# eric-zqwang/puzzlefusion-plusplus

Hardware: AMD Instinct MI355X
Metric: denoiser DDPM-step throughput (fragment*steps/s) (higher is better)
Workload: dtype f32 (GEMMs: f16x3); 1 GPU; DDPM training iteration, BASELINE configs[1]: add_noise + rotate + frozen PointNet++/VQ encode (in the loop) + DenoiserTransformer forward (dropouts on) + MSE + full backward + [encoder of iteration i+1 issued on its own stream during iteration i] AdamW; padded_slots=not evaluated (their gradient contribution is exactly zero), puzzles_per_gpu=32, fragment_slots=20, points_per_fragment=1024, valid_fragments_per_gpu=154, weights=random init, reference architecture (57.6M denoiser + 0.6M encoder params)

## Files before the change

### puzzlefusion-plusplus_amd/csrc/sa_train.hip

```cpp
#include <hip/hip_runtime.h>
#include <stdint.h>

#include "gemm_common.h"
#include "pfpp.h"
#include "pfpp_common.h"
#include "sa_common.h"

namespace {

struct SaTP {
  const float* xyz; const float* ctr; const float* feats; const int32_t* idx;
  const _Float16* wh[3]; const _Float16* wl[3];
  const float* bias[3];
  const float* am[2]; const float* aa[2];
  double* stats; int copies;
  float* y_out; float* out_max; float* out_min;
  int N, S, G;
  const float* u; int D;
  _Float16* e_hi; _Float16* e_lo;
  const int32_t* sched;
};

struct PadWalk {
  const int32_t* order;
  int G, n2, S, i, ib;
  __device__ __forceinline__ PadWalk(const int32_t* sched, int G_, int k, int S_) : order(sched), G(G_), S(S_), i(k) {
    n2 = sched ? sched[G_] : G_;
    const int r = n2 % S_;
    ib = n2 + (k >= r ? k - r : k - r + S_);
    if (i >= n2) i = ib;
  }
  __device__ __forceinline__ bool two() const { return i < n2; }
  __device__ __forceinline__ int cnt() const { return (order && i < G) ? order[2 * G + 1 + i] : 64; }
  __device__ __forceinline__ int g() const { return i < G ? (order ? order[i] : i) : G; }
  __device__ __forceinline__ void next() {
    const int j = i + S;
    i = (i < n2 && j >= n2) ? ib : j;
  }
};

__device__ __forceinline__ f32x16 bn_train_relu_t(const f32x16 acc, const float* B, const float* M, const float* A, int c0, int lhi) {
  f32x16 y;
#pragma unroll
  for (int q = 0; q < 4; ++q) {
    const float4 b4 = *reinterpret_cast<const float4*>(B + c0 + 8 * q + 4 * lhi);
    const float4 m4 = *reinterpret_cast<const float4*>(M + c0 + 8 * q + 4 * lhi);
    const float4 a4 = *reinterpret_cast<const float4*>(A + c0 + 8 * q + 4 * lhi);
    const float bv[4] = {b4.x, b4.y, b4.z, b4.w}, mv[4] = {m4.x, m4.y, m4.z, m4.w}, av[4] = {a4.x, a4.y, a4.z, a4.w};
#pragma unroll
    for (int r = 0; r < 4; ++r) {
      const float v = __builtin_fmaf(acc[4 * q + r] + bv[r], mv[r], av[r]);
      y[4 * q + r] = v > 0.0f ? v : 0.0f;
    }
  }
  return y;
}

__device__ __forceinline__ void flush_stats(double* stats, int copies, int C, int c, int lhi, double s, double q) {
  const double a = s + __shfl_xor(s, 32), b = q + __shfl_xor(q, 32);
  if (lhi == 0) {
    double* st = stats + (size_t)((blockIdx.x * 4 + (threadIdx.x >> 6)) % copies) * 2 * C;
    unsafeAtomicAdd(st + c, a);
    unsafeAtomicAdd(st + C + c, b);
  }
}

template <int C1, int C2, int C3, int STAGE>
__global__ __launch_bounds__(256, 1) void sa1_train_kernel(const SaTP p) {
  constexpr int CS = STAGE == 1 ? C1 : (STAGE == 2 ? C2 : C3);
  constexpr int NT1 = C1 / 32, NT2 = STAGE >= 2 ? C2 / 32 : 1, NT3 = STAGE >= 3 ? C3 / 32 : 1;
  __shared__ __align__(16) float B0[C1], M0[C1], A0[C1], B1[C2], M1[C2], A1[C2];
  constexpr bool LDS_SUMS = STAGE == 3;
  __shared__ double SUMS[LDS_SUMS ? 2 * (CS / 32) : 1][LDS_SUMS ? 256 : 1];
  const int tid = threadIdx.x;
  if (LDS_SUMS)
    for (int i = 0; i < 2 * (CS / 32); ++i) SUMS[i][tid] = 0.0;
  if (STAGE >= 2)
    for (int i = tid; i < C1; i += 256) { B0[i] = p.bias[0][i]; M0[i] = p.am[0][i]; A0[i] = p.aa[0][i]; }
  if (STAGE >= 3)
    for (int i = tid; i < C2; i += 256) { B1[i] = p.bias[1][i]; M1[i] = p.am[1][i]; A1[i] = p.aa[1][i]; }
  __syncthreads();

  const int lane = tid & 63, wave = tid >> 6;
  const int l31 = lane & 31, lhi = lane >> 5;

  half8 w0h[NT1], w0l[NT1];
  half8 w1h[NT2][C1 / 16], w1l[NT2][C1 / 16];
  half8 w2h[NT3][C2 / 16], w2l[NT3][C2 / 16];
#pragma unroll
  for (int t = 0; t < NT1; ++t) {
#pragma unroll
    for (int q = 0; q < 8; ++q) { w0h[t][q] = (_Float16)0.0f; w0l[t][q] = (_Float16)0.0f; }
    if (lhi == 0) {
      w0h[t] = *reinterpret_cast<const half8*>(p.wh[0] + (t * 32 + l31) * 8);
      w0l[t] = *reinterpret_cast<const half8*>(p.wl[0] + (t * 32 + l31) * 8);
    }
  }
  if (STAGE >= 2) {
#pragma unroll
    for (int t = 0; t < NT2; ++t)
#pragma unroll
      for (int ks = 0; ks < C1 / 16; ++ks) {
        w1h[t][ks] = *reinterpret_cast<const half8*>(p.wh[1] + (t * 32 + l31) * C1 + ks * 16 + lhi * 8);
        w1l[t][ks] = *reinterpret_cast<const half8*>(p.wl[1] + (t * 32 + l31) * C1 + ks * 16 + lhi * 8);
      }
  }
  if (STAGE >= 3) {
#pragma unroll
    for (int n = 0; n < NT3; ++n)
#pragma unroll
      for (int ks = 0; ks < C2 / 16; ++ks) {
        w2h[n][ks] = *reinterpret_cast<const half8*>(p.wh[2] + (n * 32 + l31) * C2 + ks * 16 + lhi * 8);
        w2l[n][ks] = *reinterpret_cast<const half8*>(p.wl[2] + (n * 32 + l31) * C2 + ks * 16 + lhi * 8);
      }
  }
  float bs[CS / 32];
  double ss[CS / 32], sq[CS / 32];
#pragma unroll
  for (int n = 0; n < CS / 32; ++n) { bs[n] = p.bias[STAGE - 1][n * 32 + l31]; ss[n] = 0.0; sq[n] = 0.0; }

  auto stat = [&](const f32x16& acc, int n, int g) {
    float s = 0.0f, q = 0.0f, mx = -__builtin_huge_valf(), mn = __builtin_huge_valf();
#pragma unroll
    for (int e = 0; e < 16; ++e) {
      const float y = acc[e] + bs[n];
      s += y;
      q = __builtin_fmaf(y, y, q);
      if (STAGE == 3) { mx = fmaxf(mx, y); mn = fminf(mn, y); }
    }
    if (LDS_SUMS) {
      SUMS[2 * n][tid] += (double)s;
      SUMS[2 * n + 1][tid] += (double)q;
    } else {
      ss[n] += (double)s;
      sq[n] += (double)q;
    }
    if (STAGE == 3) {
      mx = fmaxf(mx, __shfl_xor(mx, 32));
      mn = fminf(mn, __shfl_xor(mn, 32));
      if (lhi == 0) {
        p.out_max[(int64_t)g * C3 + n * 32 + l31] = mx;
        p.out_min[(int64_t)g * C3 + n * 32 + l31] = mn;
      }
    }
  };

  const int stride = gridDim.x * 4;
  const int g0 = blockIdx.x * 4 + wave;
  auto load_id = [&](int g) {
    const int gc = g < p.G ? g : p.G - 1;
    const int id = p.idx[(int64_t)gc * 32 + l31];
    return id < p.N ? id : p.N - 1;
  };
  auto load_pt = [&](int g, int id, float (&q)[3], float (&c)[3]) {
    const int gc = g < p.G ? g : p.G - 1;
    const int f = gc / p.S;
    const float* q3 = p.xyz + ((int64_t)f * p.N + id) * 3;
    const float* c3 = p.ctr + (int64_t)gc * 3;
#pragma unroll
    for (int d = 0; d < 3; ++d) { q[d] = q3[d]; c[d] = c3[d]; }
  };
  float q_cur[3], c_cur[3], q_nxt[3], c_nxt[3];
  int id_nxt;
  load_pt(g0, load_id(g0), q_cur, c_cur);
  id_nxt = load_id(g0 + stride);

  for (int g = g0; g < p.G; g += stride) {
    load_pt(g + stride, id_nxt, q_nxt, c_nxt);
    id_nxt = load_id(g + 2 * stride);

    half8 xh, xl;
#pragma unroll
    for (int q = 0; q < 8; ++q) { xh[q] = (_Float16)0.0f; xl[q] = (_Float16)0.0f; }
    if (lhi == 0) {
#pragma unroll
      for (int d = 0; d < 3; ++d) {
        _Float16 a, b;
        split1(__fsub_rn(q_cur[d], c_cur[d]), a, b);
        xh[d] = a; xl[d] = b;
      }
    }

    if (STAGE == 1) {
#pragma unroll
      for (int n = 0; n < NT1; ++n) {
        f32x16 acc;
#pragma unroll
        for (int e = 0; e < 16; ++e) acc[e] = 0.0f;
        acc = __builtin_amdgcn_mfma_f32_32x32x16_f16(xl, w0h[n], acc, 0, 0, 0);
        acc = __builtin_amdgcn_mfma_f32_32x32x16_f16(xh, w0l[n], acc, 0, 0, 0);
        acc = __builtin_amdgcn_mfma_f32_32x32x16_f16(xh, w0h[n], acc, 0, 0, 0);
        stat(acc, n, g);
      }
    } else {
      half8 f1h[C1 / 16], f1l[C1 / 16];
#pragma unroll
      for (int t = 0; t < NT1; ++t) {
        f32x16 acc;
#pragma unroll
        for (int e = 0; e < 16; ++e) acc[e] = 0.0f;
        acc = __builtin_amdgcn_mfma_f32_32x32x16_f16(w0h[t], xl, acc, 0, 0, 0);
        acc = __builtin_amdgcn_mfma_f32_32x32x16_f16(w0l[t], xh, acc, 0, 0, 0);
        acc = __builtin_amdgcn_mfma_f32_32x32x16_f16(w0h[t], xh, acc, 0, 0, 0);
        const f32x16 y = bn_train_relu_t(acc, B0, M0, A0, t * 32, lhi);
        half8 fh[2], fl[2];
        tile_to_fragments(y, lhi, fh, fl);
        f1h[2 * t] = fh[0]; f1h[2 * t + 1] = fh[1];
        f1l[2 * t] = fl[0]; f1l[2 * t + 1] = fl[1];
      }
      if (STAGE == 2) {
#pragma unroll
        for (int n = 0; n < NT2; ++n) {
          f32x16 acc;
#pragma unroll
          for (int e = 0; e < 16; ++e) acc[e] = 0.0f;
#pragma unroll
          for (int ks = 0; ks < C1 / 16; ++ks) {
            acc = __builtin_amdgcn_mfma_f32_32x32x16_f16(f1l[ks], w1h[n][ks], acc, 0, 0, 0);
            acc = __builtin_amdgcn_mfma_f32_32x32x16_f16(f1h[ks], w1l[n][ks], acc, 0, 0, 0);
            acc = __builtin_amdgcn_mfma_f32_32x32x16_f16(f1h[ks], w1h[n][ks], acc, 0, 0, 0);
          }
          stat(acc, n, g);
        }
      } else {
        asm volatile("" ::: "memory");
        half8 f2h[C2 / 16], f2l[C2 / 16];
#pragma unroll
        for (int t = 0; t < NT2; ++t) {
          f32x16 acc;
#pragma unroll
          for (int e = 0; e < 16; ++e) acc[e] = 0.0f;
#pragma unroll
          for (int ks = 0; ks < C1 / 16; ++ks) {
            acc = __builtin_amdgcn_mfma_f32_32x32x16_f16(w1h[t][ks], f1l[ks], acc, 0, 0, 0);
            acc = __builtin_amdgcn_mfma_f32_32x32x16_f16(w1l[t][ks], f1h[ks], acc, 0, 0, 0);
            acc = __builtin_amdgcn_mfma_f32_32x32x16_f16(w1h[t][ks], f1h[ks], acc, 0, 0, 0);
          }
          const f32x16 y = bn_train_relu_t(acc, B1, M1, A1, t * 32, lhi);
          half8 fh[2], fl[2];
          tile_to_fragments(y, lhi, fh, fl);
          f2h[2 * t] = fh[0]; f2h[2 * t + 1] = fh[1];
          f2l[2 * t] = fl[0]; f2l[2 * t + 1] = fl[1];
        }
#pragma unroll
        for (int n = 0; n < NT3; ++n) {
          f32x16 acc;
#pragma unroll
          for (int e = 0; e < 16; ++e) acc[e] = 0.0f;
#pragma unroll
          for (int ks = 0; ks < C2 / 16; ++ks) {
            acc = __builtin_amdgcn_mfma_f32_32x32x16_f16(f2l[ks], w2h[n][ks], acc, 0, 0, 0);
            acc = __builtin_amdgcn_mfma_f32_32x32x16_f16(f2h[ks], w2l[n][ks], acc, 0, 0, 0);
            acc = __builtin_amdgcn_mfma_f32_32x32x16_f16(f2h[ks], w2h[n][ks], acc, 0, 0, 0);
          }
          stat(acc, n, g);
        }
      }
    }
#pragma unroll
    for (int d = 0; d < 3; ++d) { q_cur[d] = q_nxt[d]; c_cur[d] = c_nxt[d]; }
  }
#pragma unroll
  for (int n = 0; n < CS / 32; ++n)
    flush_stats(p.stats, p.copies, CS, n * 32 + l31, lhi, LDS_SUMS ? SUMS[LDS_SUMS ? 2 * n : 0][LDS_SUMS ? tid : 0] : ss[n],
                LDS_SUMS ? SUMS[LDS_SUMS ? 2 * n + 1 : 0][LDS_SUMS ? tid : 0] : sq[n]);
}

template <int D, int C1, int C2, int STAGE>
__global__ __launch_bounds__(256, 1) void sa2_train_kernel(const SaTP p) {
  constexpr int KS0 = D / 16 + 1;
  constexpr int KP0 = D + 8;
  constexpr int LD0 = KS0 * 16 + 8, LD1 = C1 + 8;
  constexpr int CS = STAGE == 1 ? C1 : C2;
  extern __shared__ __align__(16) unsigned char sa2t_smem[];
  _Float16* W0h = reinterpret_cast<_Float16*>(sa2t_smem);
  _Float16* W0l = W0h + C1 * LD0;
  _Float16* W1h = W0l + C1 * LD0;
  _Float16* W1l = W1h + C2 * LD1;
  float* B0 = reinterpret_cast<float*>(W1l + C2 * LD1);
  float* M0 = B0 + C1;
  float* A0 = M0 + C1;

  const int tid = threadIdx.x;
  for (int i = tid; i < C1 * (LD0 / 8); i += 256) {
    const int r = i / (LD0 / 8), c8 = i - r * (LD0 / 8);
    uint4 vh = make_uint4(0, 0, 0, 0), vl = vh;
    if (c8 * 8 < KP0) {
      vh = *reinterpret_cast<const uint4*>(p.wh[0] + (size_t)r * KP0 + c8 * 8);
      vl = *reinterpret_cast<const uint4*>(p.wl[0] + (size_t)r * KP0 + c8 * 8);
    }
    *reinterpret_cast<uint4*>(W0h + r * LD0 + c8 * 8) = vh;
    *reinterpret_cast<uint4*>(W0l + r * LD0 + c8 * 8) = vl;
  }
  if (STAGE == 2) {
    for (int i = tid; i < C2 * (C1 / 8); i += 256) {
      const int r = i / (C1 / 8), c8 = i - r * (C1 / 8);
      *reinterpret_cast<uint4*>(W1h + r * LD1 + c8 * 8) = *reinterpret_cast<const uint4*>(p.wh[1] + (size_t)r * C1 + c8 * 8);
      *reinterpret_cast<uint4*>(W1l + r * LD1 + c8 * 8) = *reinterpret_cast<const uint4*>(p.wl[1] + (size_t)r * C1 + c8 * 8);
    }
    for (int i = tid; i < C1; i += 256) { B0[i] = p.bias[0][i]; M0[i] = p.am[0][i]; A0[i] = p.aa[0][i]; }
  }
  __syncthreads();

  const int lane = tid & 63, wave = tid >> 6;
  const int l31 = lane & 31, lhi = lane >> 5;

  float bs[CS / 32];
  double ss[CS / 32], sq[CS / 32];
#pragma unroll
  for (int n = 0; n < CS / 32; ++n) { bs[n] = p.bias[STAGE - 1][n * 32 + l31]; ss[n] = 0.0; sq[n] = 0.0; }

  auto split8 = [&](const float4 a, const float4 b, half8& hi, half8& lo) {
    const float x[8] = {a.x, a.y, a.z, a.w, b.x, b.y, b.z, b.w};
#pragma unroll
    for (int q = 0; q < 8; ++q) {
      _Float16 h, l;
      split1(x[q], h, l);
      hi[q] = h; lo[q] = l;
    }
  };

  const int stride = gridDim.x * 4;
  const int g0 = blockIdx.x * 4 + wave;
  auto load_ids = [&](int g, int (&id)[2]) {
    const int gc = g < p.G ? g : p.G - 1;
#pragma unroll
    for (int st = 0; st < 2; ++st) {
      const int v = p.idx[(int64_t)gc * 64 + st * 32 + l31];
      id[st] = v < p.N ? v : p.N - 1;
    }
  };
  auto load_rows = [&](int g, const int (&id)[2], float4 (&raw)[2][D / 16][2], float (&q)[2][3], float (&c)[3]) {
    const int gc = g < p.G ? g : p.G - 1;
    const int f = gc / p.S;
#pragma unroll
    for (int st = 0; st < 2; ++st) {
// ... 179 lines not shown
#pragma unroll
    for (int ks = 0; ks < K / 16; ++ks) {
      raw[ks][0] = *reinterpret_cast<const float4*>(row + ks * 16);
      raw[ks][1] = *reinterpret_cast<const float4*>(row + ks * 16 + 4);
    }
  };
  float4 raw[K / 16][2];
  PadWalk wk(p.sched, p.G, g0, stride);
  int g = wk.g(), c = wk.cnt(); wk.next();
  int g1 = wk.g(), c1 = wk.cnt(); wk.next();
  int g2 = wk.g(), c2 = wk.cnt();
  load_rows(g, 0, c, raw);
  float mx[N / 32], mn[N / 32];

  for (; g < p.G; g = g1, c = c1, g1 = g2, c1 = c2, wk.next(), g2 = wk.g(), c2 = wk.cnt()) {
    const int nh = c > 32 ? 2 : 1;
#pragma unroll 1
    for (int h = 0; h < nh; ++h) {
      asm volatile("" ::: "memory");
      half8 fh[K / 16], fl[K / 16];
#pragma unroll
      for (int ks = 0; ks < K / 16; ++ks) {
        const float4 m0 = *reinterpret_cast<const float4*>(M + ks * 16 + lhi * 8), m1 = *reinterpret_cast<const float4*>(M + ks * 16 + lhi * 8 + 4);
        const float4 a0 = *reinterpret_cast<const float4*>(A + ks * 16 + lhi * 8), a1 = *reinterpret_cast<const float4*>(A + ks * 16 + lhi * 8 + 4);
        const float mv[8] = {m0.x, m0.y, m0.z, m0.w, m1.x, m1.y, m1.z, m1.w}, av[8] = {a0.x, a0.y, a0.z, a0.w, a1.x, a1.y, a1.z, a1.w};
        const float4 r0 = raw[ks][0], r1 = raw[ks][1];
        const float x[8] = {r0.x, r0.y, r0.z, r0.w, r1.x, r1.y, r1.z, r1.w};
#pragma unroll
        for (int q = 0; q < 8; ++q) {
          const float v = fmaxf(__builtin_fmaf(x[q], mv[q], av[q]), 0.0f);
          _Float16 hh, ll;
          split1(v, hh, ll);
          fh[ks][q] = hh; fl[ks][q] = ll;
        }
      }
      if (h + 1 < nh) load_rows(g, 1, c, raw);
      else load_rows(g1, 0, c1, raw);
#pragma unroll 1
      for (int n = 0; n < N / 32; ++n) {
        f32x16 acc;
#pragma unroll
        for (int e = 0; e < 16; ++e) acc[e] = 0.0f;
#pragma unroll
        for (int ks = 0; ks < K / 16; ++ks) {
          const half8 wh = *reinterpret_cast<const half8*>(Wh + (n * 32 + l31) * LD + ks * 16 + lhi * 8);
          const half8 wl = *reinterpret_cast<const half8*>(Wl + (n * 32 + l31) * LD + ks * 16 + lhi * 8);
          acc = __builtin_amdgcn_mfma_f32_32x32x16_f16(fl[ks], wh, acc, 0, 0, 0);
          acc = __builtin_amdgcn_mfma_f32_32x32x16_f16(fh[ks], wl, acc, 0, 0, 0);
          acc = __builtin_amdgcn_mfma_f32_32x32x16_f16(fh[ks], wh, acc, 0, 0, 0);
        }
        float s = 0.0f, q = 0.0f, hi = -__builtin_huge_valf(), lo = __builtin_huge_valf();
#pragma unroll
        for (int e = 0; e < 16; ++e) {
          const float y = acc[e] + bs[n];
          s += y;
          q = __builtin_fmaf(y, y, q);
          hi = fmaxf(hi, y); lo = fminf(lo, y);
        }
        ss[n] += (double)s;
        sq[n] += (double)q;
        if (nh == 1) {
          const double y0 = lhi == 0 ? (double)(acc[0] + bs[n]) : 0.0;
          ss[n] += 32.0 * y0;
          sq[n] += 32.0 * y0 * y0;
        }
        if (h + 1 < nh) { mx[n] = hi; mn[n] = lo; }
        else {
          if (h == 1) { hi = fmaxf(hi, mx[n]); lo = fminf(lo, mn[n]); }
          hi = fmaxf(hi, __shfl_xor(hi, 32));
          lo = fminf(lo, __shfl_xor(lo, 32));
          if (lhi == 0) {
            p.out_max[(int64_t)g * N + n * 32 + l31] = hi;
            p.out_min[(int64_t)g * N + n * 32 + l31] = lo;
          }
        }
      }
    }
  }
#pragma unroll
  for (int n = 0; n < N / 32; ++n) flush_stats(p.stats, p.copies, N, n * 32 + l31, lhi, ss[n], sq[n]);
}

template <int K, int LAYER, bool UG = false, bool EVAL = false>
__global__ __launch_bounds__(256, 1) void sa_wide_train_kernel(const SaTP p, const float* __restrict__ y_in, int n_total) {
  static_assert(!UG || LAYER == 2, "the per-point table feeds the second layer");
  static_assert(!EVAL || UG, "the eval form exists for the table-fed second layer only");
  constexpr bool GATHER = LAYER == 1;
  constexpr int KS = K / 16 + (GATHER ? 1 : 0);
  constexpr int KP = GATHER ? K + 8 : K;
  constexpr int LD = KS * 16 + 8;
  constexpr int NSL = 128;
  extern __shared__ __align__(16) unsigned char saw_smem[];
  _Float16* Wh = reinterpret_cast<_Float16*>(saw_smem);
  _Float16* Wl = Wh + NSL * LD;
  float* M = reinterpret_cast<float*>(Wl + NSL * LD);
  float* A = M + K;
  const int tid = threadIdx.x;
  const int n_slices = n_total / NSL;
  const int row_wgs = gridDim.x / n_slices;
  const int slice = blockIdx.x / row_wgs, wg_row = blockIdx.x - slice * row_wgs;
  const _Float16* wh_g = p.wh[LAYER - 1] + (size_t)slice * NSL * KP;
  const _Float16* wl_g = p.wl[LAYER - 1] + (size_t)slice * NSL * KP;
  for (int i = tid; i < NSL * (LD / 8); i += 256) {
    const int r = i / (LD / 8), c8 = i - r * (LD / 8);
    uint4 vh = make_uint4(0, 0, 0, 0), vl = vh;
    if (c8 * 8 < KP) {
      vh = *reinterpret_cast<const uint4*>(wh_g + (size_t)r * KP + c8 * 8);
      vl = *reinterpret_cast<const uint4*>(wl_g + (size_t)r * KP + c8 * 8);
    }
    *reinterpret_cast<uint4*>(Wh + r * LD + c8 * 8) = vh;
    *reinterpret_cast<uint4*>(Wl + r * LD + c8 * 8) = vl;
  }
  if (!GATHER)
    for (int i = tid; i < K; i += 256) { M[i] = p.am[LAYER - 2][i]; A[i] = p.aa[LAYER - 2][i]; }
  if (UG) {
    const int kp1 = p.D + 8;
    for (int i = tid; i < 3 * K; i += 256) {
      const int d = i / K, ch = i - d * K;
      const size_t o = (size_t)ch * kp1 + p.D + d;
      (A + 5 * K)[i] = (float)p.wh[0][o] + (float)p.wl[0][o];
    }
  }
  __syncthreads();

  const int lane = tid & 63, wave = tid >> 6;
  const int l31 = lane & 31, lhi = lane >> 5;
  const int col0 = slice * NSL;
  constexpr int CPL = K / 64;
  float* AS = UG ? A + K + wave * K : A;
  float* WX = A + 5 * K;
  float bs[4];
  double ss[4], sq[4];
#pragma unroll
  for (int n = 0; n < 4; ++n) { bs[n] = p.bias[LAYER - 1] ? p.bias[LAYER - 1][col0 + n * 32 + l31] : 0.0f; ss[n] = 0.0; sq[n] = 0.0; }
  float es[EVAL ? 4 : 1], et[EVAL ? 4 : 1];
  if (EVAL) {
#pragma unroll
    for (int n = 0; n < 4; ++n) { es[n] = p.am[1][col0 + n * 32 + l31]; et[n] = p.aa[1][col0 + n * 32 + l31]; }
  }

  const int stride = row_wgs * 4;
  const int g0 = wg_row * 4 + wave;
  auto load_half = [&](int g, int half, int live, float4 (&raw)[K / 16][2], float (&q)[3], float (&c)[3]) {
    const int gc = g < p.G ? g : p.G - 1;
    if (GATHER) {
      const int f = gc / p.S;
      int id = p.idx[(int64_t)gc * 64 + half * 32 + l31];
      id = id < p.N ? id : p.N - 1;
      const float* row = p.feats + ((int64_t)f * p.N + id) * K + lhi * 8;
#pragma unroll
      for (int ks = 0; ks < K / 16; ++ks) {
        raw[ks][0] = *reinterpret_cast<const float4*>(row + ks * 16);
        raw[ks][1] = *reinterpret_cast<const float4*>(row + ks * 16 + 4);
      }
      const float* q3 = p.xyz + ((int64_t)f * p.N + id) * 3;
      const float* c3 = p.ctr + (int64_t)gc * 3;
#pragma unroll
      for (int d = 0; d < 3; ++d) { q[d] = q3[d]; c[d] = c3[d]; }
    } else if (UG) {
      const int f = gc / p.S;
      int id = p.idx[(int64_t)gc * 64 + half * 32 + l31];
      id = id < p.N ? id : p.N - 1;
      const float* row = p.u + ((int64_t)f * p.N + id) * K + lhi * 8;
#pragma unroll
      for (int ks = 0; ks < K / 16; ++ks) {
        raw[ks][0] = *reinterpret_cast<const float4*>(row + ks * 16);
        raw[ks][1] = *reinterpret_cast<const float4*>(row + ks * 16 + 4);
      }
      if (half == 0) {
        const float* c3 = p.ctr + (int64_t)gc * 3;
#pragma unroll
        for (int d = 0; d < 3; ++d) c[d] = c3[d];
      }
    } else {
      const int j = half * 32 + l31;
      const float* row = y_in + ((int64_t)gc * 64 + (j < live ? j : 0)) * K + lhi * 8;
#pragma unroll
      for (int ks = 0; ks < K / 16; ++ks) {
        raw[ks][0] = *reinterpret_cast<const float4*>(row + ks * 16);
        raw[ks][1] = *reinterpret_cast<const float4*>(row + ks * 16 + 4);
      }
    }
  };
  float4 raw[K / 16][2];
  float qx[3] = {0.f, 0.f, 0.f}, cx[3] = {0.f, 0.f, 0.f};
  PadWalk wk(EVAL ? nullptr : p.sched, p.G, g0, stride);
  int g = wk.g(), lv = wk.cnt(); wk.next();
  int g1 = wk.g(), lv1 = wk.cnt(); wk.next();
  int g2 = wk.g(), lv2 = wk.cnt();
  load_half(g, 0, lv, raw, qx, cx);

  for (; g < p.G; g = g1, lv = lv1, g1 = g2, lv1 = lv2, wk.next(), g2 = wk.g(), lv2 = wk.cnt()) {
    const int nh = lv > 32 ? 2 : 1;
    float mx[4], mn[4];
#pragma unroll
    for (int n = 0; n < 4; ++n) { mx[n] = -__builtin_huge_valf(); mn[n] = __builtin_huge_valf(); }
    if (UG) {
#pragma unroll
      for (int c = 0; c < CPL; ++c) {
        const int ch = lane * CPL + c;
        const float v = __builtin_fmaf(WX[2 * K + ch], cx[2], __builtin_fmaf(WX[K + ch], cx[1], WX[ch] * cx[0]));
        AS[ch] = __builtin_fmaf(-M[ch], v, A[ch]);
      }
    }
#pragma unroll 1
    for (int half = 0; half < nh; ++half) {
      asm volatile("" ::: "memory");
      half8 fh[KS], fl[KS];
#pragma unroll
      for (int ks = 0; ks < K / 16; ++ks) {
        const float4 r0 = raw[ks][0], r1 = raw[ks][1];
        float x[8] = {r0.x, r0.y, r0.z, r0.w, r1.x, r1.y, r1.z, r1.w};
        if (!GATHER) {
          const float4 m0 = *reinterpret_cast<const float4*>(M + ks * 16 + lhi * 8), m1 = *reinterpret_cast<const float4*>(M + ks * 16 + lhi * 8 + 4);
          const float4 a0 = *reinterpret_cast<const float4*>(AS + ks * 16 + lhi * 8), a1 = *reinterpret_cast<const float4*>(AS + ks * 16 + lhi * 8 + 4);
          const float mv[8] = {m0.x, m0.y, m0.z, m0.w, m1.x, m1.y, m1.z, m1.w}, av[8] = {a0.x, a0.y, a0.z, a0.w, a1.x, a1.y, a1.z, a1.w};
#pragma unroll
          for (int q8 = 0; q8 < 8; ++q8) x[q8] = fmaxf(__builtin_fmaf(x[q8], mv[q8], av[q8]), 0.0f);
        }
#pragma unroll
        for (int q8 = 0; q8 < 8; ++q8) {
          _Float16 h, l;
          split1(x[q8], h, l);
          fh[ks][q8] = h; fl[ks][q8] = l;
        }
      }
      if (GATHER) {
#pragma unroll
        for (int q8 = 0; q8 < 8; ++q8) { fh[KS - 1][q8] = (_Float16)0.0f; fl[KS - 1][q8] = (_Float16)0.0f; }
        if (lhi == 0) {
#pragma unroll
          for (int d = 0; d < 3; ++d) {
            _Float16 a, b;
            split1(__fsub_rn(qx[d], cx[d]), a, b);
            fh[KS - 1][d] = a; fl[KS - 1][d] = b;
          }
        }
      }
      if (half + 1 < nh) load_half(g, 1, lv, raw, qx, cx); else load_half(g1, 0, lv1, raw, qx, cx);
      f32x16 acc[4];
#pragma unroll
      for (int n = 0; n < 4; ++n)
#pragma unroll
        for (int e = 0; e < 16; ++e) acc[n][e] = 0.0f;
#pragma unroll
      for (int ks = 0; ks < KS; ++ks) {
        half8 wh[4], wl[4];
#pragma unroll
        for (int n = 0; n < 4; ++n) {
          wh[n] = *reinterpret_cast<const half8*>(Wh + (n * 32 + l31) * LD + ks * 16 + lhi * 8);
          wl[n] = *reinterpret_cast<const half8*>(Wl + (n * 32 + l31) * LD + ks * 16 + lhi * 8);
        }
#pragma unroll
        for (int n = 0; n < 4; ++n) acc[n] = __builtin_amdgcn_mfma_f32_32x32x16_f16(fl[ks], wh[n], acc[n], 0, 0, 0);
#pragma unroll
        for (int n = 0; n < 4; ++n) acc[n] = __builtin_amdgcn_mfma_f32_32x32x16_f16(fh[ks], wl[n], acc[n], 0, 0, 0);
#pragma unroll
        for (int n = 0; n < 4; ++n) acc[n] = __builtin_amdgcn_mfma_f32_32x32x16_f16(fh[ks], wh[n], acc[n], 0, 0, 0);
      }
      if (EVAL) {
#pragma unroll
        for (int n = 0; n < 4; ++n) {
          const int64_t o0 = ((int64_t)g * 64 + half * 32 + 4 * lhi) * n_total + col0 + n * 32 + l31;
#pragma unroll
          for (int e = 0; e < 16; ++e) {
            const float v = fmaxf(__builtin_fmaf(acc[n][e] + bs[n], es[n], et[n]), 0.0f);
            _Float16 h, l;
            split1(v, h, l);
            const int64_t o = o0 + (int64_t)((e & 3) + 8 * (e >> 2)) * n_total;
            p.e_hi[o] = h; p.e_lo[o] = l;
          }
        }
        continue;
      }
#pragma unroll
      for (int n = 0; n < 4; ++n) {
        float s = 0.0f, q = 0.0f;
        float* orow = LAYER < 3 ? p.y_out + ((int64_t)g * 64 + half * 32 + 4 * lhi) * n_total + col0 + n * 32 + l31 : nullptr;
#pragma unroll
        for (int e = 0; e < 16; ++e) {
          const float y = acc[n][e] + bs[n];
          s += y;
          q = __builtin_fmaf(y, y, q);
          if (LAYER == 3) { mx[n] = fmaxf(mx[n], y); mn[n] = fminf(mn[n], y); }
          else if (half * 32 + 4 * lhi + (e & 3) + 8 * (e >> 2) < lv) orow[(int64_t)((e & 3) + 8 * (e >> 2)) * n_total] = y;
        }
        ss[n] += (double)s;
        sq[n] += (double)q;
        if (nh == 1) {
          const double y0 = lhi == 0 ? (double)(acc[n][0] + bs[n]) : 0.0;
          ss[n] += 32.0 * y0;
          sq[n] += 32.0 * y0 * y0;
        }
      }
    }
    if (LAYER == 3) {
#pragma unroll
      for (int n = 0; n < 4; ++n) {
        const float a = fmaxf(mx[n], __shfl_xor(mx[n], 32)), b = fminf(mn[n], __shfl_xor(mn[n], 32));
        if (lhi == 0) {
          p.out_max[(int64_t)g * n_total + col0 + n * 32 + l31] = a;
          p.out_min[(int64_t)g * n_total + col0 + n * 32 + l31] = b;
        }
      }
    }
  }
#pragma unroll
  for (int n = 0; n < 4; ++n)
    if (!EVAL) flush_stats(p.stats, p.copies, n_total, col0 + n * 32 + l31, lhi, ss[n], sq[n]);
}

template <int K>
__global__ __launch_bounds__(256) void sa_first_stats_kernel(const SaTP p) {
  constexpr int CPL = K / 64;
  typedef float vecf __attribute__((ext_vector_type(CPL)));
  __shared__ double red[2][4][K];
  const int tid = threadIdx.x, lane = tid & 63, wave = tid >> 6;
  const int kp1 = p.D + 8;
  float uw[CPL][3];
#pragma unroll
  for (int c = 0; c < CPL; ++c)
#pragma unroll
    for (int d = 0; d < 3; ++d) {
      const size_t o = (size_t)(lane * CPL + c) * kp1 + p.D + d;
      uw[c][d] = (float)p.wh[0][o] + (float)p.wl[0][o];
    }
  double ss[CPL], sq[CPL];
#pragma unroll
  for (int c = 0; c < CPL; ++c) { ss[c] = 0.0; sq[c] = 0.0; }
  for (int g = blockIdx.x * 4 + wave; g < p.G; g += gridDim.x * 4) {
    const int f = g / p.S;
    int id = p.idx[(int64_t)g * 64 + lane];
    id = id < p.N ? id : p.N - 1;
    const float* c3 = p.ctr + (int64_t)g * 3;
    const float cx = c3[0], cy = c3[1], cz = c3[2];
    float v[CPL], s[CPL], q[CPL];
#pragma unroll
    for (int c = 0; c < CPL; ++c) {
      v[c] = __builtin_fmaf(uw[c][2], cz, __builtin_fmaf(uw[c][1], cy, uw[c][0] * cx));
      s[c] = 0.0f; q[c] = 0.0f;
    }
    const float* ub = p.u + (int64_t)f * p.N * K + lane * CPL;
    const int id0 = __shfl(id, 0);
    const unsigned long long live = __ballot(id != id0);
    const int runs = live ? (64 - __clzll(live) + 15) >> 4 : 1;
    const vecf r0 = *reinterpret_cast<const vecf*>(ub + (int64_t)id0 * K);
    float y0[CPL];
#pragma unroll
    for (int c = 0; c < CPL; ++c) y0[c] = r0[c] - v[c];
#pragma unroll 1
    for (int j0 = 0; j0 < runs * 16; j0 += 16) {
#pragma unroll
      for (int jj = 0; jj < 16; ++jj) {
        const int idj = __shfl(id, j0 + jj);
        const vecf r = *reinterpret_cast<const vecf*>(ub + (int64_t)idj * K);
#pragma unroll
        for (int c = 0; c < CPL; ++c) {
          const float y = r[c] - v[c];
          s[c] += y;
          q[c] = __builtin_fmaf(y, y, q[c]);
        }
      }
    }
    const double np = (double)(64 - runs * 16);
#pragma unroll
    for (int c = 0; c < CPL; ++c) { ss[c] += (double)s[c] + np * (double)y0[c]; sq[c] += (double)q[c] + np * (double)y0[c] * (double)y0[c]; }
  }
#pragma unroll
  for (int c = 0; c < CPL; ++c) { red[0][wave][lane * CPL + c] = ss[c]; red[1][wave][lane * CPL + c] = sq[c]; }
  __syncthreads();
  double* st = p.stats + (size_t)(blockIdx.x % p.copies) * 2 * K;
  for (int i = tid; i < 2 * K; i += 256) {
    const int w = i / K, c = i - w * K;
    unsafeAtomicAdd(st + w * K + c, (red[w][0][c] + red[w][1][c]) + (red[w][2][c] + red[w][3][c]));
  }
// ... 171 lines not shown

unsigned persistent_grid(int G, int per, int64_t cap) {
  const int64_t need = (G + per - 1) / per;
  return (unsigned)(need < cap ? need : cap);
}

unsigned rows_grid(int64_t cap, int n_total) {
  const int n_slices = n_total / 128;
  cap = cap / (8 * n_slices) * (8 * n_slices);
  return (unsigned)(cap < n_slices ? n_slices : cap);
}

constexpr size_t sa_lds(int rows, int k, int n_vec) { return (size_t)2 * rows * (k + 8) * sizeof(_Float16) + (size_t)n_vec * k * sizeof(float); }
constexpr int gathered(int d) { return (d / 16 + 1) * 16; }

template <auto KERN, typename... Args>
int launch_sa(const char* instantiation, unsigned grid, unsigned block, size_t smem, hipStream_t st, Args... args) {
  static const KernelName name("%s", instantiation);
  report_kernel(name);
  if (smem) (void)pfpp_allow_dyn_lds<KERN>((int)smem);
  hipLaunchKernelGGL(KERN, dim3(grid), dim3(block), smem, st, args...);
  return pfpp::check_launch("pfpp_sa_train_stage");
}

}

extern "C" int pfpp_sa_train_stage(const pfpp_sa_train_args* a, pfpp_stream_t stream) {
  pfpp_gemm_detail::pl::last_kernel[0] = 0;
  PFPP_REQUIRE(a, "null args");
  PFPP_REQUIRE(a->xyz && a->new_xyz && a->idx && a->stats, "null pointer");
  PFPP_REQUIRE(a->F >= 0 && a->N > 0 && a->S > 0 && a->stats_copies >= 1, "bad sizes");
  PFPP_REQUIRE(a->stage >= 1 && a->stage <= 3, "stage out of range (1..3)");
  const int L = a->stage;
  const bool lvl1 = a->feats == nullptr;
  const bool table = a->u_in && L <= 2;
  const SaLevel level = lvl1 ? SaLevel::NoFeatures : a->D == 256 ? SaLevel::Feats256 : SaLevel::Feats128;
  if (table) {
    PFPP_REQUIRE(!lvl1, "the per-point table belongs to a level with input features");
    PFPP_SUPPORTED(a->ns == 64 && ((a->D == 128 && a->C1 == 128 && a->C2 == 128) || (a->D == 256 && a->C1 == 256 && a->C2 == 256)),
                   "per-point first layer: nsample 64, (128 -> 128 -> 128) or (256 -> 256 -> 256) only");
    PFPP_REQUIRE(a->w_hi[0] && a->w_lo[0] && pfpp::aligned16(a->u_in), "first-layer planes / table alignment");
    PFPP_REQUIRE(a->F * a->S < (1ll << 25), "too many neighbourhoods");
    PFPP_REQUIRE(L == 1 || (a->w_hi[1] && a->w_lo[1] && a->bias[1] && pfpp::aligned16(a->w_hi[1]) && pfpp::aligned16(a->w_lo[1]) && a->a_mul[0] &&
                            a->a_add[0] && a->y_out && pfpp::aligned16(a->y_out)), "second-layer operands / first-layer affine / y_out missing");
  } else if (level == SaLevel::Feats256) {
    PFPP_SUPPORTED(a->ns == 64 && a->C1 == 256 && a->C2 == 256 && a->C3 == 512, "wide train-mode level: nsample 64, 256 features, widths 256/256/512 only");
    PFPP_REQUIRE(a->w_hi[L - 1] && a->w_lo[L - 1] && a->bias[L - 1] && pfpp::aligned16(a->w_hi[L - 1]) && pfpp::aligned16(a->w_lo[L - 1]),
                 "weights / bias of the layer this stage computes are missing");
    PFPP_REQUIRE(L == 1 || (a->a_mul[L - 2] && a->a_add[L - 2] && a->y_in && pfpp::aligned16(a->y_in)), "the previous layer's rows / affine are missing");
    PFPP_REQUIRE(L == 3 ? (a->out_max && a->out_min) : (a->y_out != nullptr), "output missing");
    PFPP_REQUIRE(pfpp::aligned16(a->feats) && a->F * a->S < (1ll << 25), "alignment / too many neighbourhoods");
    PFPP_SUPPORTED(!(a->sched && L == 1), "the grouped first layer of the wide level takes no padding schedule (use the per-point table: u_in)");
  } else {
    const bool rows3 = !lvl1 && L == 3;
    for (int i = rows3 ? 2 : 0; i < L; ++i) {
      PFPP_REQUIRE(a->w_hi[i] && a->w_lo[i] && a->bias[i], "weights / bias of a layer this stage computes are missing");
      PFPP_REQUIRE(pfpp::aligned16(a->w_hi[i]) && pfpp::aligned16(a->w_lo[i]), "planes must be 16-byte aligned");
    }
    for (int i = rows3 ? 1 : 0; i + 1 < L; ++i)
      PFPP_REQUIRE(a->a_mul[i] && a->a_add[i], "finalised BatchNorm affine of an earlier layer is missing");
    if (lvl1) {
      PFPP_SUPPORTED(!a->sched, "no padding schedule for the 32-neighbour level");
      PFPP_SUPPORTED(a->ns == 32 && a->C1 == 64 && a->C2 == 64 && a->C3 == 128, "train-mode chain without features: nsample 32, widths 64/64/128 only");
      PFPP_REQUIRE(L < 3 || (a->out_max && a->out_min), "stage 3 writes the per-neighbourhood max and min");
      PFPP_REQUIRE(a->F * a->S < (1ll << 31), "too many neighbourhoods");
    } else {
      PFPP_SUPPORTED(a->ns == 64 && a->D == 128 && a->C1 == 128 && a->C2 == 128 && (L < 3 || a->C3 == 256),
                     "train-mode chain with features: nsample 64, 128 features, widths 128/128/256 only");
      PFPP_REQUIRE(L < 2 || (a->y_out && pfpp::aligned16(a->y_out)), "stage 2 writes / stage 3 reads the raw layer-2 rows");
      PFPP_REQUIRE(L < 3 || (a->out_max && a->out_min), "stage 3 writes the per-neighbourhood max and min");
      PFPP_REQUIRE(pfpp::aligned16(a->feats), "16-byte alignment");
      PFPP_REQUIRE(a->F * a->S < (1ll << 25), "too many neighbourhoods");
      PFPP_SUPPORTED(!a->sched || L == 3, "stages 1 and 2 take the padding schedule only in their table-fed form (u_in)");
    }
  }
  if (a->F == 0) return PFPP_OK;

  const SaTP p = fill_sa(a, table);
  const int64_t cap = a->max_workgroups > 0 ? a->max_workgroups : 256;
  const unsigned per4 = persistent_grid(p.G, 4, cap);
  const float* const no_rows = nullptr;
  hipStream_t st = pfpp::as_stream(stream);
  switch (choose_sa_stage((int)a->D, L, table, level)) {
    case SaKern::Sa1Stage1: return launch_sa<sa1_train_kernel<64, 64, 128, 1>>("sa1_train_kernel<64, 64, 128, 1>", per4, 256, 0, st, p);
    case SaKern::Sa1Stage2: return launch_sa<sa1_train_kernel<64, 64, 128, 2>>("sa1_train_kernel<64, 64, 128, 2>", per4, 256, 0, st, p);
    case SaKern::Sa1Stage3: return launch_sa<sa1_train_kernel<64, 64, 128, 3>>("sa1_train_kernel<64, 64, 128, 3>", per4, 256, 0, st, p);
    case SaKern::Sa2Stage1:
      return launch_sa<sa2_train_kernel<128, 128, 128, 1>>("sa2_train_kernel<128, 128, 128, 1>", per4, 256, sa_lds(128, gathered(128), 0), st, p);
    case SaKern::Sa2Stage2:
      return launch_sa<sa2_train_kernel<128, 128, 128, 2>>("sa2_train_kernel<128, 128, 128, 2>", per4, 256,
                                                           sa_lds(128, gathered(128), 0) + sa_lds(128, 128, 3), st, p);
    case SaKern::Rows8:
      return launch_sa<sa_rows8_train_kernel<128, 256>>("sa_rows8_train_kernel<128, 256>", persistent_grid(p.G, 8, cap), 512, sa_lds(256, 128, 2), st, p);
    case SaKern::FirstStats128:
      return launch_sa<sa_first_stats_kernel<128>>("sa_first_stats_kernel<128>", persistent_grid(p.G, 4, 4 * cap), 256, 0, st, p);
    case SaKern::FirstStats256:
      return launch_sa<sa_first_stats_kernel<256>>("sa_first_stats_kernel<256>", persistent_grid(p.G, 4, 4 * cap), 256, 0, st, p);
    case SaKern::Table128:
      return launch_sa<sa_wide_train_kernel<128, 2, true>>("sa_wide_train_kernel<128, 2, true, false>", rows_grid(cap, 128), 256, sa_lds(128, 128, 9), st, p, no_rows, 128);
    case SaKern::Table256:
      return launch_sa<sa_wide_train_kernel<256, 2, true>>("sa_wide_train_kernel<256, 2, true, false>", rows_grid(cap, 256), 256, sa_lds(128, 256, 9), st, p, no_rows, 256);
    case SaKern::Wide1:
      return launch_sa<sa_wide_train_kernel<256, 1>>("sa_wide_train_kernel<256, 1, false, false>", rows_grid(cap, 256), 256, sa_lds(128, gathered(256), 0) + 2 * 256 * sizeof(float), st, p, a->y_in, 256);
    case SaKern::Wide2:
      return launch_sa<sa_wide_train_kernel<256, 2>>("sa_wide_train_kernel<256, 2, false, false>", rows_grid(cap, 256), 256, sa_lds(128, 256, 2), st, p, a->y_in, 256);
    case SaKern::Wide3:
      return launch_sa<sa_wide_train_kernel<256, 3>>("sa_wide_train_kernel<256, 3, false, false>", rows_grid(cap, 512), 256, sa_lds(128, 256, 2), st, p, a->y_in, 512);
  }
  return PFPP_EINVAL;
}

extern "C" int pfpp_sa_mlp2_table_p(const float* u, const float* new_xyz, const int32_t* idx, const void* w0_hi, const void* w0_lo,
                                    const void* w1_hi, const void* w1_lo, const float* s0, const float* t0, const float* s1,
                                    const float* t1, const pfpp_planes* out, int64_t F, int64_t N, int64_t S, int64_t ns, int64_t D,
                                    int64_t C1, int64_t C2, int64_t max_workgroups, pfpp_stream_t stream) {
  PFPP_REQUIRE(u && new_xyz && idx && w0_hi && w0_lo && w1_hi && w1_lo && s0 && t0 && s1 && t1 && pfpp_planes_ok(out) && out, "null pointer");
  PFPP_SUPPORTED(ns == 64 && D == 128 && C1 == 128 && C2 == 128, "table-fed eval level: nsample 64, 128 features, widths 128/128 only");
  PFPP_SUPPORTED(out->scale == 1.0f, "unit plane scale only");
  PFPP_REQUIRE(pfpp::aligned16(u) && pfpp::aligned16(w1_hi) && pfpp::aligned16(w1_lo) && F >= 0 && N > 0 && S > 0 && F * S < (1ll << 25),
               "alignment / sizes");
  if (F == 0) return PFPP_OK;
  SaTP p = {};
  p.ctr = new_xyz; p.idx = idx;
  p.wh[0] = (const _Float16*)w0_hi; p.wl[0] = (const _Float16*)w0_lo;
  p.wh[1] = (const _Float16*)w1_hi; p.wl[1] = (const _Float16*)w1_lo;
  p.am[0] = s0; p.aa[0] = t0; p.am[1] = s1; p.aa[1] = t1;
  p.N = (int)N; p.S = (int)S; p.G = (int)(F * S);
  p.u = u; p.D = (int)D;
  p.e_hi = (_Float16*)out->hi; p.e_lo = (_Float16*)out->lo;
  int64_t cap = max_workgroups > 0 ? max_workgroups : 256;
  cap = cap / 8 * 8;
  if (cap < 1) cap = 1;
  const int64_t need = (p.G + 3) / 4;
  if (need < cap) cap = need;
  constexpr size_t smem = (size_t)2 * 128 * (128 + 8) * sizeof(_Float16) + (2 + 4 + 3) * 128 * sizeof(float);
  (void)pfpp_allow_dyn_lds<sa_wide_train_kernel<128, 2, true, true>>((int)smem);
  hipLaunchKernelGGL((sa_wide_train_kernel<128, 2, true, true>), dim3((unsigned)cap), dim3(256), smem, pfpp::as_stream(stream), p, (const float*)nullptr, 128);
  return pfpp::check_launch("pfpp_sa_mlp2_table_p");
}

extern "C" int pfpp_sa_table_planes(const float* u, const float* new_xyz, const int32_t* idx, const void* w0_hi, const void* w0_lo,
                                    const float* s0, const float* t0, const pfpp_planes* out, int64_t F, int64_t N, int64_t S, int64_t ns,
                                    int64_t D, int64_t C1, pfpp_stream_t stream) {
  PFPP_REQUIRE(u && new_xyz && idx && w0_hi && w0_lo && s0 && t0 && out && pfpp_planes_ok(out), "null pointer");
  PFPP_SUPPORTED(ns == 64 && ((D == 256 && C1 == 256) || (D == 128 && C1 == 128)), "table-fed first layer: nsample 64, (256 -> 256) or (128 -> 128)");
  PFPP_SUPPORTED(out->scale == 1.0f, "unit plane scale only");
  PFPP_REQUIRE(pfpp::aligned16(u) && F >= 0 && N > 0 && S > 0 && F * S < (1ll << 25), "alignment / sizes");
  if (F == 0) return PFPP_OK;
  SaTP p = {};
  p.ctr = new_xyz; p.idx = idx;
  p.wh[0] = (const _Float16*)w0_hi; p.wl[0] = (const _Float16*)w0_lo;
  p.am[0] = s0; p.aa[0] = t0;
  p.N = (int)N; p.S = (int)S; p.G = (int)(F * S);
  p.u = u; p.D = (int)D;
  p.e_hi = (_Float16*)out->hi; p.e_lo = (_Float16*)out->lo;
  const int64_t need = (p.G + 3) / 4;
  const unsigned grid = (unsigned)(need < 2048 ? need : 2048);
  hipStream_t st = pfpp::as_stream(stream);
  if (D == 256) hipLaunchKernelGGL((sa_table_apply_kernel<256>), dim3(grid), dim3(256), 0, st, p);
  else hipLaunchKernelGGL((sa_table_apply_kernel<128>), dim3(grid), dim3(256), 0, st, p);
  return pfpp::check_launch("pfpp_sa_table_planes");
}
```

Before: 26340 fragment*steps/s.

## Raise SA training kernels to two waves per SIMD via LDS weights and N-tiling

The sa1 stage kernels now launch with a two-blocks-per-CU bound, and stage 3 moves its third-layer weights from registers into padded LDS. Grid caps are raised to match. The 128-wide table-fed wide kernel also gets a two-block bound and processes one 32-column output tile at a time instead of four, which cuts accumulator register pressure. The aim is better latency hiding through higher occupancy, at the cost of extra LDS reads per MFMA and the loss of cross-tile ILP in the wide kernel.

```diff
diff --git a/puzzlefusion-plusplus_amd/csrc/sa_train.hip b/puzzlefusion-plusplus_amd/csrc/sa_train.hip
--- a/puzzlefusion-plusplus_amd/csrc/sa_train.hip
+++ b/puzzlefusion-plusplus_amd/csrc/sa_train.hip
@@ -66,19 +66,27 @@
 }
 
 template <int C1, int C2, int C3, int STAGE>
-__global__ __launch_bounds__(256, 1) void sa1_train_kernel(const SaTP p) {
+__global__ __launch_bounds__(256, 2) void sa1_train_kernel(const SaTP p) {
   constexpr int CS = STAGE == 1 ? C1 : (STAGE == 2 ? C2 : C3);
   constexpr int NT1 = C1 / 32, NT2 = STAGE >= 2 ? C2 / 32 : 1, NT3 = STAGE >= 3 ? C3 / 32 : 1;
   __shared__ __align__(16) float B0[C1], M0[C1], A0[C1], B1[C2], M1[C2], A1[C2];
   constexpr bool LDS_SUMS = STAGE == 3;
+  constexpr int LD2 = C2 + 8;
   __shared__ double SUMS[LDS_SUMS ? 2 * (CS / 32) : 1][LDS_SUMS ? 256 : 1];
+  __shared__ __align__(16) _Float16 W2h[STAGE == 3 ? C3 * LD2 : 8], W2l[STAGE == 3 ? C3 * LD2 : 8];
   const int tid = threadIdx.x;
   if (LDS_SUMS)
     for (int i = 0; i < 2 * (CS / 32); ++i) SUMS[i][tid] = 0.0;
   if (STAGE >= 2)
     for (int i = tid; i < C1; i += 256) { B0[i] = p.bias[0][i]; M0[i] = p.am[0][i]; A0[i] = p.aa[0][i]; }
-  if (STAGE >= 3)
+  if (STAGE >= 3) {
     for (int i = tid; i < C2; i += 256) { B1[i] = p.bias[1][i]; M1[i] = p.am[1][i]; A1[i] = p.aa[1][i]; }
+    for (int i = tid; i < C3 * (C2 / 8); i += 256) {
+      const int r = i / (C2 / 8), c8 = i - r * (C2 / 8);
+      *reinterpret_cast<uint4*>(W2h + r * LD2 + c8 * 8) = *reinterpret_cast<const uint4*>(p.wh[2] + (size_t)r * C2 + c8 * 8);
+      *reinterpret_cast<uint4*>(W2l + r * LD2 + c8 * 8) = *reinterpret_cast<const uint4*>(p.wl[2] + (size_t)r * C2 + c8 * 8);
+    }
+  }
   __syncthreads();
 
   const int lane = tid & 63, wave = tid >> 6;
@@ -86,7 +94,6 @@
 
   half8 w0h[NT1], w0l[NT1];
   half8 w1h[NT2][C1 / 16], w1l[NT2][C1 / 16];
-  half8 w2h[NT3][C2 / 16], w2l[NT3][C2 / 16];
 #pragma unroll
   for (int t = 0; t < NT1; ++t) {
 #pragma unroll
@@ -103,15 +110,6 @@
       for (int ks = 0; ks < C1 / 16; ++ks) {
         w1h[t][ks] = *reinterpret_cast<const half8*>(p.wh[1] + (t * 32 + l31) * C1 + ks * 16 + lhi * 8);
         w1l[t][ks] = *reinterpret_cast<const half8*>(p.wl[1] + (t * 32 + l31) * C1 + ks * 16 + lhi * 8);
-      }
-  }
-  if (STAGE >= 3) {
-#pragma unroll
-    for (int n = 0; n < NT3; ++n)
-#pragma unroll
-      for (int ks = 0; ks < C2 / 16; ++ks) {
-        w2h[n][ks] = *reinterpret_cast<const half8*>(p.wh[2] + (n * 32 + l31) * C2 + ks * 16 + lhi * 8);
-        w2l[n][ks] = *reinterpret_cast<const half8*>(p.wl[2] + (n * 32 + l31) * C2 + ks * 16 + lhi * 8);
       }
   }
   float bs[CS / 32];
@@ -249,9 +247,11 @@
           for (int e = 0; e < 16; ++e) acc[e] = 0.0f;
 #pragma unroll
           for (int ks = 0; ks < C2 / 16; ++ks) {
-            acc = __builtin_amdgcn_mfma_f32_32x32x16_f16(f2l[ks], w2h[n][ks], acc, 0, 0, 0);
-            acc = __builtin_amdgcn_mfma_f32_32x32x16_f16(f2h[ks], w2l[n][ks], acc, 0, 0, 0);
-            acc = __builtin_amdgcn_mfma_f32_32x32x16_f16(f2h[ks], w2h[n][ks], acc, 0, 0, 0);
+            const half8 wh = *reinterpret_cast<const half8*>(W2h + (n * 32 + l31) * LD2 + ks * 16 + lhi * 8);
+            const half8 wl = *reinterpret_cast<const half8*>(W2l + (n * 32 + l31) * LD2 + ks * 16 + lhi * 8);
+            acc = __builtin_amdgcn_mfma_f32_32x32x16_f16(f2l[ks], wh, acc, 0, 0, 0);
+            acc = __builtin_amdgcn_mfma_f32_32x32x16_f16(f2h[ks], wl, acc, 0, 0, 0);
+            acc = __builtin_amdgcn_mfma_f32_32x32x16_f16(f2h[ks], wh, acc, 0, 0, 0);
           }
           stat(acc, n, g);
         }
@@ -597,7 +597,7 @@
 }
 
 template <int K, int LAYER, bool UG = false, bool EVAL = false>
-__global__ __launch_bounds__(256, 1) void sa_wide_train_kernel(const SaTP p, const float* __restrict__ y_in, int n_total) {
+__global__ __launch_bounds__(256, (K == 128 && !EVAL) ? 2 : 1) void sa_wide_train_kernel(const SaTP p, const float* __restrict__ y_in, int n_total) {
   static_assert(!UG || LAYER == 2, "the per-point table feeds the second layer");
   static_assert(!EVAL || UG, "the eval form exists for the table-fed second layer only");
   constexpr bool GATHER = LAYER == 1;
@@ -605,6 +605,8 @@
   constexpr int KP = GATHER ? K + 8 : K;
   constexpr int LD = KS * 16 + 8;
   constexpr int NSL = 128;
+  constexpr bool TWO_WAVES = K == 128 && !EVAL;
+  constexpr int NT = TWO_WAVES ? 1 : 4;
   extern __shared__ __align__(16) unsigned char saw_smem[];
   _Float16* Wh = reinterpret_cast<_Float16*>(saw_smem);
   _Float16* Wl = Wh + NSL * LD;
@@ -753,59 +755,65 @@
         }
       }
       if (half + 1 < nh) load_half(g, 1, lv, raw, qx, cx); else load_half(g1, 0, lv1, raw, qx, cx);
-      f32x16 acc[4];
-#pragma unroll
-      for (int n = 0; n < 4; ++n)
-#pragma unroll
-        for (int e = 0; e < 16; ++e) acc[n][e] = 0.0f;
-#pragma unroll
-      for (int ks = 0; ks < KS; ++ks) {
-        half8 wh[4], wl[4];
-#pragma unroll
-        for (int n = 0; n < 4; ++n) {
-          wh[n] = *reinterpret_cast<const half8*>(Wh + (n * 32 + l31) * LD + ks * 16 + lhi * 8);
-          wl[n] = *reinterpret_cast<const half8*>(Wl + (n * 32 + l31) * LD + ks * 16 + lhi * 8);
-        }
-#pragma unroll
-        for (int n = 0; n < 4; ++n) acc[n] = __builtin_amdgcn_mfma_f32_32x32x16_f16(fl[ks], wh[n], acc[n], 0, 0, 0);
-#pragma unroll
-        for (int n = 0; n < 4; ++n) acc[n] = __builtin_amdgcn_mfma_f32_32x32x16_f16(fh[ks], wl[n], acc[n], 0, 0, 0);
-#pragma unroll
-        for (int n = 0; n < 4; ++n) acc[n] = __builtin_amdgcn_mfma_f32_32x32x16_f16(fh[ks], wh[n], acc[n], 0, 0, 0);
-      }
-      if (EVAL) {
-#pragma unroll
-        for (int n = 0; n < 4; ++n) {
-          const int64_t o0 = ((int64_t)g * 64 + half * 32 + 4 * lhi) * n_total + col0 + n * 32 + l31;
-#pragma unroll
-          for (int e = 0; e < 16; ++e) {
-            const float v = fmaxf(__builtin_fmaf(acc[n][e] + bs[n], es[n], et[n]), 0.0f);
-            _Float16 h, l;
-            split1(v, h, l);
-            const int64_t o = o0 + (int64_t)((e & 3) + 8 * (e >> 2)) * n_total;
-            p.e_hi[o] = h; p.e_lo[o] = l;
+#pragma unroll
+      for (int n0 = 0; n0 < 4; n0 += NT) {
+        if (NT < 4) asm volatile("" ::: "memory");
+        f32x16 acc[NT];
+#pragma unroll
+        for (int j = 0; j < NT; ++j)
+#pragma unroll
+          for (int e = 0; e < 16; ++e) acc[j][e] = 0.0f;
+#pragma unroll
+        for (int ks = 0; ks < KS; ++ks) {
+          half8 wh[NT], wl[NT];
+#pragma unroll
+          for (int j = 0; j < NT; ++j) {
+            wh[j] = *reinterpret_cast<const half8*>(Wh + ((n0 + j) * 32 + l31) * LD + ks * 16 + lhi * 8);
+            wl[j] = *reinterpret_cast<const half8*>(Wl + ((n0 + j) * 32 + l31) * LD + ks * 16 + lhi * 8);
           }
-        }
-        continue;
-      }
-#pragma unroll
-      for (int n = 0; n < 4; ++n) {
-        float s = 0.0f, q = 0.0f;
-        float* orow = LAYER < 3 ? p.y_out + ((int64_t)g * 64 + half * 32 + 4 * lhi) * n_total + col0 + n * 32 + l31 : nullptr;
-#pragma unroll
-        for (int e = 0; e < 16; ++e) {
-          const float y = acc[n][e] + bs[n];
-          s += y;
-          q = __builtin_fmaf(y, y, q);
-          if (LAYER == 3) { mx[n] = fmaxf(mx[n], y); mn[n] = fminf(mn[n], y); }
-          else if (half * 32 + 4 * lhi + (e & 3) + 8 * (e >> 2) < lv) orow[(int64_t)((e & 3) + 8 * (e >> 2)) * n_total] = y;
-        }
-        ss[n] += (double)s;
-        sq[n] += (double)q;
-        if (nh == 1) {
-          const double y0 = lhi == 0 ? (double)(acc[n][0] + bs[n]) : 0.0;
-          ss[n] += 32.0 * y0;
-          sq[n] += 32.0 * y0 * y0;
+#pragma unroll
+          for (int j = 0; j < NT; ++j) acc[j] = __builtin_amdgcn_mfma_f32_32x32x16_f16(fl[ks], wh[j], acc[j], 0, 0, 0);
+#pragma unroll
+          for (int j = 0; j < NT; ++j) acc[j] = __builtin_amdgcn_mfma_f32_32x32x16_f16(fh[ks], wl[j], acc[j], 0, 0, 0);
+#pragma unroll
+          for (int j = 0; j < NT; ++j) acc[j] = __builtin_amdgcn_mfma_f32_32x32x16_f16(fh[ks], wh[j], acc[j], 0, 0, 0);
+        }
+        if (EVAL) {
+#pragma unroll
+          for (int j = 0; j < NT; ++j) {
+            const int n = n0 + j;
+            const int64_t o0 = ((int64_t)g * 64 + half * 32 + 4 * lhi) * n_total + col0 + n * 32 + l31;
+#pragma unroll
+            for (int e = 0; e < 16; ++e) {
+              const float v = fmaxf(__builtin_fmaf(acc[j][e] + bs[n], es[n], et[n]), 0.0f);
+              _Float16 h, l;
+              split1(v, h, l);
+              const int64_t o = o0 + (int64_t)((e & 3) + 8 * (e >> 2)) * n_total;
+              p.e_hi[o] = h; p.e_lo[o] = l;
+            }
+          }
+        } else {
+#pragma unroll
+          for (int j = 0; j < NT; ++j) {
+            const int n = n0 + j;
+            float s = 0.0f, q = 0.0f;
+            float* orow = LAYER < 3 ? p.y_out + ((int64_t)g * 64 + half * 32 + 4 * lhi) * n_total + col0 + n * 32 + l31 : nullptr;
+#pragma unroll
+            for (int e = 0; e < 16; ++e) {
+              const float y = acc[j][e] + bs[n];
+              s += y;
+              q = __builtin_fmaf(y, y, q);
+              if (LAYER == 3) { mx[n] = fmaxf(mx[n], y); mn[n] = fminf(mn[n], y); }
+              else if (half * 32 + 4 * lhi + (e & 3) + 8 * (e >> 2) < lv) orow[(int64_t)((e & 3) + 8 * (e >> 2)) * n_total] = y;
+            }
+            ss[n] += (double)s;
+            sq[n] += (double)q;
+            if (nh == 1) {
+              const double y0 = lhi == 0 ? (double)(acc[j][0] + bs[n]) : 0.0;
+              ss[n] += 32.0 * y0;
+              sq[n] += 32.0 * y0 * y0;
+            }
+          }
         }
       }
     }
@@ -1143,9 +1151,12 @@
   const float* const no_rows = nullptr;
   hipStream_t st = pfpp::as_stream(stream);
   switch (choose_sa_stage((int)a->D, L, table, level)) {
-    case SaKern::Sa1Stage1: return launch_sa<sa1_train_kernel<64, 64, 128, 1>>("sa1_train_kernel<64, 64, 128, 1>", per4, 256, 0, st, p);
-    case SaKern::Sa1Stage2: return launch_sa<sa1_train_kernel<64, 64, 128, 2>>("sa1_train_kernel<64, 64, 128, 2>", per4, 256, 0, st, p);
-    case SaKern::Sa1Stage3: return launch_sa<sa1_train_kernel<64, 64, 128, 3>>("sa1_train_kernel<64, 64, 128, 3>", per4, 256, 0, st, p);
+    case SaKern::Sa1Stage1:
+      return launch_sa<sa1_train_kernel<64, 64, 128, 1>>("sa1_train_kernel<64, 64, 128, 1>", persistent_grid(p.G, 4, 4 * cap), 256, 0, st, p);
+    case SaKern::Sa1Stage2:
+      return launch_sa<sa1_train_kernel<64, 64, 128, 2>>("sa1_train_kernel<64, 64, 128, 2>", persistent_grid(p.G, 4, 2 * cap), 256, 0, st, p);
+    case SaKern::Sa1Stage3:
+      return launch_sa<sa1_train_kernel<64, 64, 128, 3>>("sa1_train_kernel<64, 64, 128, 3>", persistent_grid(p.G, 4, 2 * cap), 256, 0, st, p);
     case SaKern::Sa2Stage1:
       return launch_sa<sa2_train_kernel<128, 128, 128, 1>>("sa2_train_kernel<128, 128, 128, 1>", per4, 256, sa_lds(128, gathered(128), 0), st, p);
     case SaKern::Sa2Stage2:
@@ -1158,7 +1169,7 @@
     case SaKern::FirstStats256:
       return launch_sa<sa_first_stats_kernel<256>>("sa_first_stats_kernel<256>", persistent_grid(p.G, 4, 4 * cap), 256, 0, st, p);
     case SaKern::Table128:
-      return launch_sa<sa_wide_train_kernel<128, 2, true>>("sa_wide_train_kernel<128, 2, true, false>", rows_grid(cap, 128), 256, sa_lds(128, 128, 9), st, p, no_rows, 128);
+      return launch_sa<sa_wide_train_kernel<128, 2, true>>("sa_wide_train_kernel<128, 2, true, false>", rows_grid(2 * cap, 128), 256, sa_lds(128, 128, 9), st, p, no_rows, 128);
     case SaKern::Table256:
       return launch_sa<sa_wide_train_kernel<256, 2, true>>("sa_wide_train_kernel<256, 2, true, false>", rows_grid(cap, 256), 256, sa_lds(128, 256, 9), st, p, no_rows, 256);
     case SaKern::Wide1:
```

Result: no change. 26190 fragment*steps/s (-0.5%).
